# palantir/k8s-spark-scheduler

Hardware: AMD Instinct MI355X
Metric: gang-fit decisions/sec at 10k nodes x 1k pending apps (+ p99 Filter latency: fifo_filter) (higher is better)
Workload: dtype int64; 1 GPU; independent batch, tightly-pack, 10000 nodes x 1000 pending apps per GPU, 3-D (cpu milli, mem bytes, gpu) int64, SURVEY.md 8d/C2 distributions, seed 0x5EED0010; nodes=10000, apps_per_gpu=1000, algo=tightly-pack, mode=independent, batches_in_flight=11, regime=streamed_tickets (resident worker), backend=none, rccl_ranks=0

## Files before the change

### include/gangfit.h

```cpp
#ifndef GANGFIT_H
#define GANGFIT_H

#include <stddef.h>
#include <stdint.h>

#ifdef __cplusplus
extern "C" {
#endif

#define GF_VERSION 300

#define GF_OK 0
#define GF_ERR_NO_DEVICE (-1)
#define GF_ERR_HIP (-2)
#define GF_ERR_INVALID (-3)
#define GF_ERR_CAPACITY (-4)
#define GF_ERR_STATE (-5)
#define GF_ERR_UNSUPPORTED (-6)

#define GF_NO_NODE 0xFFFFFFFFu
#define GF_MAX_K (1 << 20)
#define GF_MAX_ABS_QUANTITY (INT64_C(1) << 62)

typedef enum gf_algo {
// ... 198 lines not shown

int gf_hbm_probe(gf_ctx *ctx, uint64_t bytes, uint32_t iters, double *read_gb_per_s, double *copy_gb_per_s);

int gf_launch_floor(gf_ctx *ctx, void *stream, uint32_t iters, float *us_per_launch);

typedef struct gf_worker_batch {
    uint32_t n_apps;
    uint32_t flags;
    const gf_app *d_apps;
    gf_result *d_results;
    uint32_t *d_exec_nodes;
    uint64_t exec_nodes_len;
} gf_worker_batch;
#define GF_WORKER_HOST_OUTPUTS 1u
#define GF_WORKER_LEAVE_AFTER 2u
int gf_worker_fit(gf_ctx *ctx, gf_algo algo, uint32_t n_apps, const gf_app *apps, gf_result *results, uint32_t *exec_nodes,
                  uint64_t exec_nodes_cap);
int gf_worker_submit_dev(gf_ctx *ctx, gf_algo algo, uint32_t n_batches, const gf_worker_batch *batches, uint64_t *first_ticket);
int gf_worker_wait(gf_ctx *ctx, uint64_t first_ticket, uint32_t n_tickets);
int gf_worker_stop(gf_ctx *ctx);
int gf_worker_stats(gf_ctx *ctx, uint64_t out[4]);
int gf_worker_geometry(gf_ctx *ctx, uint32_t out[2]);
int gf_worker_row_stats(gf_ctx *ctx, uint64_t out[3]);
int gf_call_phases(gf_ctx *ctx, double out_us[5]);
int gf_worker_kernel_time(gf_ctx *ctx, float *ms, uint64_t *tickets);

typedef struct gf_device_info {
    char name[128];
    char arch[64];
    int32_t compute_units;
    int32_t lds_bytes_per_cu;
    int32_t wavefront_size;
    int32_t clock_khz;
    int64_t hbm_bytes;
} gf_device_info;
int gf_device_info_get(gf_ctx *ctx, gf_device_info *out);

#ifdef __cplusplus
}
#endif
#endif
```

### k8s-spark-scheduler_amd/csrc/gangfit_api_worker.cpp

```cpp
#include "gangfit_ctx.h"

using namespace gfapi;

namespace gfapi {

constexpr uint32_t kRing = gangfit::kWorkerRing;

inline uint64_t host_load(const unsigned long long* p) { return __atomic_load_n(p, __ATOMIC_ACQUIRE); }
inline void host_store(unsigned long long* p, uint64_t v) { __atomic_store_n(p, (unsigned long long)v, __ATOMIC_RELEASE); }

int worker_alloc(gf_ctx* ctx) {
    gf_ctx::Worker& w = ctx->worker;
    if (w.allocated) return GF_OK;
    GF_HIP(ctx, hipSetDevice(ctx->device));
    void* hp = nullptr;
    GF_HIP(ctx, hipHostMalloc(&hp, sizeof(gangfit::WorkerHostCtl), hipHostMallocMapped | hipHostMallocCoherent));
    std::memset(hp, 0, sizeof(gangfit::WorkerHostCtl));
    void* hd = nullptr;
    if (hipHostGetDevicePointer(&hd, hp, 0) != hipSuccess) {
        (void)hipHostFree(hp);
        return fail(ctx, GF_ERR_HIP, "the worker's control block cannot be mapped to the device");
    }
    void* dp = nullptr;
    if (hipMalloc(&dp, sizeof(gangfit::WorkerDevCtl)) != hipSuccess ||
// ... 361 lines not shown
}

int gf_worker_geometry(gf_ctx* ctx, uint32_t out[2]) {
    if (!ctx || !out) return GF_ERR_INVALID;
    std::lock_guard<std::recursive_mutex> lock(ctx->mu);
    out[0] = ctx->worker.cur_sets;
    out[1] = ctx->worker.cur_blocks_per_set;
    return GF_OK;
}

int gf_worker_row_stats(gf_ctx* ctx, uint64_t out[3]) {
    if (!ctx || !out) return GF_ERR_INVALID;
    std::lock_guard<std::recursive_mutex> lock(ctx->mu);
    out[0] = out[1] = out[2] = 0;
    const gf_ctx::Worker& w = ctx->worker;
    if (!w.allocated) return GF_OK;
    GF_HIP(ctx, hipSetDevice(ctx->device));
    unsigned long long h[3] = {0, 0, 0};
    GF_HIP(ctx, hipMemcpy(h, w.d->rows, sizeof(h), hipMemcpyDeviceToHost));
    for (int i = 0; i < 3; ++i) out[i] = h[i];
    return GF_OK;
}

int gf_worker_kernel_time(gf_ctx* ctx, float* ms, uint64_t* tickets) {
    if (!ctx || !ms || !tickets) return GF_ERR_INVALID;
    std::lock_guard<std::recursive_mutex> lock(ctx->mu);
    const gf_ctx::Worker& w = ctx->worker;
    if (!w.allocated || w.launches == 0 || (w.running && w.launches == 1))
        return fail(ctx, GF_ERR_STATE, "no launch of the worker has finished yet (gf_worker_stop first)");
    if (!w.running) worker_elapsed(ctx->worker);
    *ms = w.last_ms;
    *tickets = w.last_tickets;
    return GF_OK;
}

}
```

### k8s-spark-scheduler_amd/csrc/gangfit_device.h

```cpp
#pragma once

#include <hip/hip_runtime.h>
#include <stdint.h>

#include <optional>

#include "gangfit.h"
#include "gangfit_worker_rounds.h"
#include "gangfit_worker_rows.h"

namespace gangfit {

struct NodeTable {
    int64_t* cpu;
    int64_t* mem;
    int64_t* gpu;
    const uint32_t* slot_node;
    const uint32_t* dslot;
    const uint32_t* node_slot;
    const int64_t* cmax;
    const uint64_t* xmask;
    const uint64_t* dmask;
    uint32_t n_chunks;
    uint32_t n_x;
// ... 96 lines not shown
constexpr uint32_t kWorkerInline = 16;
constexpr int kWorkerWaves = 16;
constexpr uint32_t kWorkerCountStride = 64;

struct WorkerTicket {
    unsigned long long word[8];
};
static_assert(sizeof(WorkerTicket) == 64, "one cache line per ticket");
__host__ __device__ inline unsigned long long worker_tag(unsigned long long ticket) { return ((ticket + 1ull) & 0x7FFFull) | 0x8000ull; }

struct WorkerHostCtl {
    unsigned long long posted;
    unsigned long long stop;
    unsigned long long pad0[6];
    unsigned long long consumed;
    unsigned long long state;
    unsigned long long pad1[6];
    unsigned long long done[kWorkerRing];
    WorkerTicket ring[kWorkerRing];
};

struct WorkerDevCtl {
    unsigned long long quit;
    unsigned long long rows[3];
    unsigned long long pad0[4];
    uint32_t count[kWorkerRing * kWorkerCountStride];
    WorkerTicket ring[kWorkerRing];
};

struct WorkerArgs {
    WorkerHostCtl* host;
    WorkerDevCtl* dev;
    unsigned long long generation;
    unsigned long long first_ticket;
    unsigned long long idle_ticks;
    unsigned long long leave_after;
    uint32_t* scratch;
    unsigned long long scratch_stride;
    uint32_t sets;
    uint32_t blocks_per_set;
    ScanStats* stats;
    uint32_t n_inline;
    uint32_t stride_mul;
    unsigned long long inline_words[kWorkerInline][6];
    ZoneTable zones;
    const int64_t* sched;
    uint32_t stride_shift;
    uint32_t pad_stride;
// ... 390 lines not shown
```

### k8s-spark-scheduler_amd/csrc/gangfit_worker.inc

```







__device__ __forceinline__ unsigned long long sys_load(const unsigned long long* p) {
    return __hip_atomic_load(p, __ATOMIC_RELAXED, __HIP_MEMORY_SCOPE_SYSTEM);
}
__device__ __forceinline__ void sys_store(unsigned long long* p, unsigned long long v) {
    __hip_atomic_store(p, v, __ATOMIC_RELAXED, __HIP_MEMORY_SCOPE_SYSTEM);
}

__device__ __forceinline__ App app_from_lanes(unsigned long long w) {
    App r;
    r.drv0 = (int64_t)read_lane((int64_t)w, 0);
    r.drv1 = (int64_t)read_lane((int64_t)w, 1);
    r.drv2 = (int64_t)read_lane((int64_t)w, 2);
    r.exe0 = (int64_t)read_lane((int64_t)w, 3);
    r.exe1 = (int64_t)read_lane((int64_t)w, 4);
    r.exe2 = (int64_t)read_lane((int64_t)w, 5);
    const uint64_t kf = (uint64_t)read_lane((int64_t)w, 6);
    r.k = (int32_t)(uint32_t)kf;
    r.flags = (uint32_t)(kf >> 32);
// ... 95 lines not shown
    r.node = read_lane(dnode, r.fl);
    r.found = true;
    return r;
}
static_assert(rows::kCapClamp == GF_MAX_K && rows::kRowLen == (uint32_t)kWave && rows::kRows <= (uint32_t)kWave, "lane = entry");

constexpr int kWorkerCounting = 100 + (int)GF_ALGO_TIGHTLY_PACK;
template <int WHICH>
__global__ __launch_bounds__(kWave* kWorkerWaves, 4) void fit_worker_kernel(NodeTable T, SparseTable G, WorkerArgs W) {
    constexpr int ALGO = WHICH == kWorkerCounting ? (int)GF_ALGO_TIGHTLY_PACK : WHICH;
    constexpr bool COUNT = WHICH != (int)GF_ALGO_TIGHTLY_PACK;
    constexpr bool kZoned = ALGO == GF_ALGO_SINGLE_AZ_TIGHTLY_PACK || ALGO == GF_ALGO_AZ_AWARE_TIGHTLY_PACK;
    constexpr int kInner = kZoned ? (int)GF_ALGO_TIGHTLY_PACK : ALGO;
    __shared__ uint32_t s_cnt[8];
    __shared__ uint32_t s_round[kWorkerWaves];
    __shared__ unsigned long long s_next[8];
    __shared__ unsigned long long s_g0[5][kWave];
    constexpr bool kNarrow = ALGO == GF_ALGO_TIGHTLY_PACK;
    __shared__ int32_t s_g0n[kNarrow ? 3 : 1][kWave];
    constexpr bool kRowsOn = WHICH == (int)GF_ALGO_TIGHTLY_PACK;
    constexpr uint32_t kRowsN = kRowsOn ? rows::kRows : 1u;
    struct RowsLds {
        uint32_t dir[kWave];
        int32_t key[3][kWave];
        uint32_t slot[kRowsN][kWave];
        uint32_t node[kRowsN][kWave];
        int32_t cap[kRowsN][kWave];
    };
    __shared__ RowsLds s_rows[1];
    __shared__ unsigned long long s_row_stat[3];
    __shared__ uint32_t s_left;
    const int lane = lane_id();
    const uint32_t wave = __builtin_amdgcn_readfirstlane(threadIdx.x >> 6);
    if (blockIdx.x == 0) {
        if (wave != 0) return;
        unsigned long long consumed = W.first_ticket;
        unsigned long long last = wall_clock64();
        if (lane == 0) sys_store(&W.host->state, 1ull);
        for (;;) {
            const unsigned long long posted = sys_load(&W.host->posted);
            const unsigned long long stop = sys_load(&W.host->stop);
            if (posted > consumed) {
                while (consumed < posted) {
                    unsigned long long w4[4];
#pragma unroll
                    for (int q = 0; q < 4; ++q) {
                        const unsigned long long t = consumed + (unsigned long long)(lane >> 3) + 8ull * (unsigned long long)q;
                        w4[q] = 0;
                        if (t < posted)
                            w4[q] = sys_load(reinterpret_cast<const unsigned long long*>(&W.host->ring[(uint32_t)(t % kWorkerRing)]) + (lane & 7));
                    }
#pragma unroll
                    for (int q = 0; q < 4; ++q) {
// ... 17 lines not shown
                }
                asm volatile("s_waitcnt vmcnt(0)" ::: "memory");
                if (lane == 0) sys_store(&W.host->state, 2ull);
                return;
            }
            __builtin_amdgcn_s_sleep(8);
        }
    }
    const uint32_t b = blockIdx.x - 1u;
    const uint32_t set = b / W.blocks_per_set, bs = b % W.blocks_per_set;
    const uint32_t app_stride = W.blocks_per_set * kWorkerWaves;
    const rounds::StrideDiv sdiv{W.stride_mul, W.stride_shift};
    unsigned long long t = W.first_ticket + (unsigned long long)((set + W.sets - (uint32_t)(W.first_ticket % W.sets)) % W.sets);
    GlobalView V{T.cpu, T.mem, T.gpu, T.cmax, T.cmax + T.n_chunks, T.cmax + 2 * (size_t)T.n_chunks, T.xmask, T.dmask,
                 T.n_chunks};
    Orders O{T.slot_node, T.dslot, T.n_x, T.n_d, T.d_identity != 0};
    const bool merged = T.d_identity != 0 && kInner != GF_ALGO_MINIMAL_FRAGMENTATION;
    constexpr uint32_t kCountSlots = 8;
    constexpr uint32_t kRoundGone = 0xFFFFFFFFu;
    if (threadIdx.x < kCountSlots) s_cnt[threadIdx.x] = 0;
    if (threadIdx.x < 8) s_next[threadIdx.x] = 0ull;
    if (threadIdx.x < (uint32_t)kWorkerWaves) s_round[threadIdx.x] = 0;
    if constexpr (kRowsOn) {
        if (threadIdx.x < kRowsN) s_rows[0].dir[threadIdx.x] = rows::kEmpty;
        if (threadIdx.x < 3) s_row_stat[threadIdx.x] = 0ull;
        if (threadIdx.x == 0) s_left = 0u;
    }
    const bool narrow_table = kNarrow && T.nquad != nullptr;
    bool rows_live = kRowsOn && merged &&
                           (W.leave_after == 0ull || W.leave_after - W.first_ticket >= (unsigned long long)rows::kRowSightings * W.sets);
    if (wave == 0) {
        const Group0 g = load_group0(V, O, lane);
        s_g0[0][lane] = (unsigned long long)g.m0;
        s_g0[1][lane] = (unsigned long long)g.m1;
        s_g0[2][lane] = (unsigned long long)g.m2;
        s_g0[3][lane] = g.dcand;
        s_g0[4][lane] = g.xcand;
        if constexpr (kNarrow) {
            if (narrow_table) {
                s_g0n[0][lane] = NarrowView::scale_max(g.m0, T.nunit[0]);
                s_g0n[1][lane] = NarrowView::scale_max(g.m1, T.nunit[1]);
                s_g0n[2][lane] = NarrowView::scale_max(g.m2, T.nunit[2]);
            }
        }
    }
    const NarrowView VN(InWorkerKernel{}, T.nquad, T.xmask, T.dmask, T.n_chunks);
    const int64_t unit_l = T.nunit[lane % 3 == 0 ? 0 : (lane % 3 == 1 ? 1 : 2)];
    const double rcp_l = kNarrow ? fast_rcp((double)unit_l) : 0.0;
    __syncthreads();
    constexpr bool kG0Regs = kNarrow;
    Group0T<int32_t> g0n_regs{};
    if constexpr (kG0Regs) {
        if (narrow_table) {
            g0n_regs.m0 = s_g0n[0][lane];
            g0n_regs.m1 = s_g0n[1][lane];
            g0n_regs.m2 = s_g0n[2][lane];
            g0n_regs.dcand = s_g0[3][lane];
            g0n_regs.xcand = s_g0[4][lane];
        }
    }
    typedef __attribute__((address_space(1))) const gf_app glb_app;
    typedef __attribute__((address_space(1))) gf_result glb_result;
    typedef __attribute__((address_space(1))) uint32_t glb_u32w;
    constexpr unsigned long long kPtrMask = 0x0000FFFFFFFFFFFFull;
    constexpr bool kRecords = ALGO != GF_ALGO_MINIMAL_FRAGMENTATION;
    auto load_words = [&](unsigned long long tt) {
        const unsigned long long* line = reinterpret_cast<const unsigned long long*>(&W.dev->ring[(uint32_t)(tt % kWorkerRing)]);
        unsigned long long w = 0;
        if (lane < 6) w = __hip_atomic_load(line + lane, __ATOMIC_RELAXED, __HIP_MEMORY_SCOPE_AGENT);
        return w;
    };
// ... 97 lines not shown
        uint32_t* scratch = priv + W.scratch_stride;
        const bool direct = ALGO == GF_ALGO_TIGHTLY_PACK && ((w5 >> 32) & 1ull) == 0;
        uint32_t mine = 0;
        for (uint32_t a = kRecords ? app_index(i_cur) : first_app; kRecords ? i_cur < total : a < n_apps;
             a = kRecords ? a : a + app_stride) {
            if constexpr (kRecords) {
                if (a >= n_apps) {
                    i_cur = grab(round);
                    a = app_index(i_cur);
                    if (i_cur < total && a < n_apps) wrec = load_record(apps, a);
                    continue;
                }
            }
            unsigned long long xvis = 0, dvis = 0;
            Decision dec;
            int32_t app_k = 0;
            uint64_t app_off = 0;
            bool decided = false;
            int build_row = -1;
            const uint32_t* placed = nullptr;
            if constexpr (kNarrow) {
                NarrowApp napp;
                auto sparse_serves = [&]() { return worker_kernargs_here()->G.n_x != 0u && O.d_identity; };
                if (narrow_table && scale_record(wrec, lane, unit_l, rcp_l, napp)) {
                if constexpr (kRowsOn) {
                    if (rows_live && napp.k > 0) {
                        RowsLds& R = s_rows[0];
                        int rl = lane;
                        GF_HERE(rl);
                        uint32_t st = rows::kEmpty;
                        bool same = false;
                        if ((uint32_t)rl < kRowsN) {
                            st = __hip_atomic_load(&R.dir[rl], __ATOMIC_ACQUIRE, __HIP_MEMORY_SCOPE_WORKGROUP);
                            const int32_t k0 = R.key[0][rl], k1 = R.key[1][rl], k2 = R.key[2][rl];
                            same = (bool)((int)rows::dir_has_key(st) & (int)(k0 == napp.exe0) & (int)(k1 == napp.exe1) & (int)(k2 == napp.exe2));
                        }
                        const uint64_t hit = __ballot(same);
                        bool served = false;
                        if (hit) {
                            const int e = __ffsll((unsigned long long)hit) - 1;
                            const uint32_t ste = read_lane(st, e);
                            if (rows::dir_ready(ste)) {
                                const RowDriver rd = wave_row_driver(VN, O, napp, g0n_regs, lane);
                                if (rd.found) {
                                    const int32_t c_ds = read_lane(cap3(rd.d0 - napp.drv0, rd.d1 - napp.drv1, rd.d2 - napp.drv2, napp), rd.fl);
                                    const int32_t cp = rows::entry_cap(R.slot[e][rl], R.cap[e][rl], rd.ds, c_ds);
                                    const uint32_t node = R.node[e][rl];
                                    const int32_t incl = wave_inclusive_scan(cp);
                                    if (rows::served((int64_t)read_lane(incl, kWave - 1), napp.k)) {
                                        const int64_t start = (int64_t)(incl - cp);
                                        emit_runs((direct ? exec_nodes : priv) + napp.exec_off, start, rows::run_of(start, cp, napp.k), node,
                                                  lane, direct);
                                        app_k = napp.k;
                                        app_off = napp.exec_off;
                                        dec.feasible = true;
                                        dec.ds = rd.ds;
                                        dec.pass1 = 0;
                                        dec.ds_node = rd.node;
                                        decided = served = true;
                                    }
                                }
                            } else if (rows::dir_counting(ste)) {
                                uint32_t old = 0;
                                if (lane == 0) old = __hip_atomic_fetch_add(&R.dir[e], 1u, __ATOMIC_RELAXED, __HIP_MEMORY_SCOPE_WORKGROUP);
                                if (rows::dir_sighting_builds((uint32_t)__builtin_amdgcn_readfirstlane(old))) build_row = e;
                            }
                        } else {
                            const uint64_t empty = __ballot((uint32_t)rl < kRowsN && st == rows::kEmpty);
                            const uint64_t claimed = __ballot(st == rows::kClaimed);
                            if (empty == 0ull && claimed == 0ull &&
                                __hip_atomic_load(&s_row_stat[0], __ATOMIC_RELAXED, __HIP_MEMORY_SCOPE_WORKGROUP) == 0ull)
                                rows_live = false;
                            if (empty != 0ull && claimed == 0ull && lane == 0) {
                                const int e = __ffsll((unsigned long long)empty) - 1;
                                uint32_t expect = rows::kEmpty;
                                if (__hip_atomic_compare_exchange_strong(&R.dir[e], &expect, rows::kClaimed, __ATOMIC_RELAXED, __ATOMIC_RELAXED,
                                                                         __HIP_MEMORY_SCOPE_WORKGROUP)) {
                                    R.key[0][e] = napp.exe0;
                                    R.key[1][e] = napp.exe1;
                                    R.key[2][e] = napp.exe2;
                                    __hip_atomic_store(&R.dir[e], rows::kFirstSighting, __ATOMIC_RELEASE, __HIP_MEMORY_SCOPE_WORKGROUP);
                                }
                            }
                        }
                        if (lane == 0)
                            __hip_atomic_fetch_add(&s_row_stat[served ? 1 : 2], 1ull, __ATOMIC_RELAXED, __HIP_MEMORY_SCOPE_WORKGROUP);
                    }
                }
                if (!decided && !(napp.exe2 > 0 && napp.k > 0 && sparse_serves())) {
                    Group0T<int32_t> g0n = g0n_regs;
                    if constexpr (!kG0Regs) {
                        g0n.m0 = s_g0n[0][lane];
                        g0n.m1 = s_g0n[1][lane];
                        g0n.m2 = s_g0n[2][lane];
                        g0n.dcand = s_g0[3][lane];
                        g0n.xcand = s_g0[4][lane];
                    }
                    app_k = napp.k;
                    app_off = napp.exec_off;
                    dec = wave_decide<ALGO, NarrowView, false>(VN, O, napp, (direct ? exec_nodes : priv) + app_off, scratch + app_off,
                                                               scratch + half + app_off, lane, xvis, dvis, &g0n, nullptr, direct);
                    if (dec.feasible && dec.ds_node == GF_NO_NODE) dec.ds_node = VN.node_of(dec.ds);
                    decided = true;
// ... 31 lines not shown
                }
            }
            if (dec.feasible && !direct) {
                if constexpr (kZoned) {
                    for (int32_t i = lane; i < app_k; i += kWave)
                        __hip_atomic_store(exec_nodes + app_off + i, T.slot_node[placed[i]], __ATOMIC_RELAXED, __HIP_MEMORY_SCOPE_SYSTEM);
                } else {
                    for (int32_t i = lane; i < app_k; i += kWave)
                        __hip_atomic_store(exec_nodes + app_off + i, priv[app_off + i], __ATOMIC_RELAXED,
                                           __HIP_MEMORY_SCOPE_SYSTEM);
                }
            }
            if (lane < 2) {
                if (dec.feasible && dec.ds_node == GF_NO_NODE) dec.ds_node = T.slot_node[dec.ds];
                const unsigned long long lo = (unsigned long long)(uint32_t)(dec.feasible ? 1 : 0) |
                                              ((unsigned long long)(dec.feasible ? dec.ds_node : GF_NO_NODE) << 32);
                const unsigned long long hi = (unsigned long long)(dec.feasible ? (uint32_t)app_k : 0u) | (1ull << 32);
                __hip_atomic_store(reinterpret_cast<unsigned long long*>(results + a) + lane, lane == 0 ? lo : hi, __ATOMIC_RELAXED,
                                   __HIP_MEMORY_SCOPE_SYSTEM);
            }
            if constexpr (kRowsOn) {
                if (__builtin_expect(build_row >= 0, 0)) {
                    NarrowApp b;
                    (void)scale_record(wrec, lane, unit_l, rcp_l, b);
                    b.k = rows::kCapClamp;
                    RowsLds& R = s_rows[0];
                    int rl = lane;
                    GF_HERE(rl);
                    R.slot[build_row][rl] = GF_NO_NODE;
                    R.node[build_row][rl] = GF_NO_NODE;
                    R.cap[build_row][rl] = 0;
                    const uint32_t xc = (O.n_x + kWave - 1) / kWave;
                    const uint64_t lt_mask = (1ull << lane) - 1ull;
                    uint32_t fill = 0;
                    for (uint32_t g = 0; g * kWave < xc && fill < rows::kRowLen; ++g) {
                        uint64_t cand;
                        uint64_t m = chunk_group_mask<false>(VN, g, xc, b.exe0, b.exe1, b.exe2, lane, cand);
                        while (m != 0ull && fill < rows::kRowLen) {
                            const int bit = __ffsll((unsigned long long)m) - 1;
                            const uint32_t c = g * kWave + (uint32_t)bit;
                            m &= m - 1;
                            const uint32_t j = c * kWave + lane;
                            const uint64_t in_m = (uint64_t)read_lane((int64_t)cand, bit) & low_lanes(chunk_len(O.n_x, c * kWave, kWave));
                            int32_t a0 = 0, a1 = 0, a2 = 0;
                            uint32_t node = 0;
                            if (lane_in(in_m)) VN.load(j, a0, a1, a2, node);
                            const uint64_t fm = ge3_mask(a0, a1, a2, b.exe0, b.exe1, b.exe2) & in_m;
                            const uint32_t pos = fill + (uint32_t)__popcll((unsigned long long)(fm & lt_mask));
                            if (lane_in(fm) && pos < rows::kRowLen) {
                                R.slot[build_row][pos] = j;
                                R.node[build_row][pos] = node;
                                R.cap[build_row][pos] = cap3(a0, a1, a2, b);
                            }
                            fill += (uint32_t)__popcll((unsigned long long)fm);
                        }
                    }
                    __builtin_amdgcn_fence(__ATOMIC_RELEASE, "workgroup");
                    if (lane == 0) {
                        __hip_atomic_fetch_add(&s_row_stat[0], 1ull, __ATOMIC_RELAXED, __HIP_MEMORY_SCOPE_WORKGROUP);
                        __hip_atomic_fetch_or(&R.dir[build_row], rows::kReadyBit, __ATOMIC_RELEASE, __HIP_MEMORY_SCOPE_WORKGROUP);
                    }
                }
            }
            ++mine;
            if constexpr (kRecords) {
                i_cur = grab(round);
                a = app_index(i_cur);
                if (i_cur < total && a < n_apps) wrec = load_record(apps, a);
            }
        }
        const unsigned long long t_next = t + W.sets;
        const bool have_next = words_valid(w_next, t_next);
        unsigned long long wrec_next = 0;
        uint32_t i_next = 0;
        const uint32_t bsr_n = rounds::next_block(bsr, W.blocks_per_set);
        const gf_app* apps_n = nullptr;
        uint64_t w5_n = 0;
        uint32_t rows_n = 0;
        if (kRecords && have_next) {
// ... 26 lines not shown
                            sys_store(&W.host->done[slot], t + 1ull);
                        }
                    }
                }
            }
        }
        ++round;
        if (lane == 0) __hip_atomic_store(&s_round[wave], round, __ATOMIC_RELAXED, __HIP_MEMORY_SCOPE_WORKGROUP);
        t = t_next;
        w_cur = w_next;
        have_cur = have_next;
        wrec = wrec_next;
        i_cur = i_next;
        grabbed_cur = kRecords && have_next;
        bsr = bsr_n;
        apps = apps_n;
        w5 = w5_n;
        rows = rows_n;
    }
    if (lane == 0) __hip_atomic_store(&s_round[wave], kRoundGone, __ATOMIC_RELAXED, __HIP_MEMORY_SCOPE_WORKGROUP);
    if constexpr (kRowsOn) {
        uint32_t left = 0;
        if (lane == 0) left = __hip_atomic_fetch_add(&s_left, 1u, __ATOMIC_ACQ_REL, __HIP_MEMORY_SCOPE_WORKGROUP);
        if ((uint32_t)__builtin_amdgcn_readfirstlane(left) == (uint32_t)kWorkerWaves - 1u && lane < 3) {
            const unsigned long long n = __hip_atomic_load(&s_row_stat[lane], __ATOMIC_RELAXED, __HIP_MEMORY_SCOPE_WORKGROUP);
            if (n != 0ull) __hip_atomic_fetch_add(&W.dev->rows[lane], n, __ATOMIC_RELAXED, __HIP_MEMORY_SCOPE_AGENT);
        }
    }
}
```

### k8s-spark-scheduler_amd/csrc/gangfit_worker_rows.h

```cpp
#pragma once
#include <cstdint>

#if defined(__HIPCC__)
#define GF_ROWS_FN __host__ __device__ inline
#else
#define GF_ROWS_FN inline
#endif

namespace gangfit {
namespace rows {

constexpr uint32_t kRowLen = 64;
constexpr uint32_t kRows = 40;
constexpr uint32_t kRowSightings = 4;
constexpr int32_t kCapClamp = 1 << 20;


constexpr uint32_t kEmpty = 0u, kClaimed = 1u, kFirstSighting = 2u, kReadyBit = 0x80000000u;
GF_ROWS_FN bool dir_ready(uint32_t w) { return (w & kReadyBit) != 0u; }
GF_ROWS_FN bool dir_has_key(uint32_t w) { return w >= kFirstSighting; }
GF_ROWS_FN bool dir_counting(uint32_t w) { return w >= kFirstSighting && w <= kRowSightings; }
GF_ROWS_FN bool dir_sighting_builds(uint32_t old) { return old == kRowSightings; }

GF_ROWS_FN int32_t entry_cap(uint32_t slot, int32_t cap, uint32_t ds, int32_t c_ds) { return slot == ds ? c_ds : cap; }
GF_ROWS_FN bool served(int64_t total, int32_t k) { return k >= 1 && total >= (int64_t)k; }
GF_ROWS_FN int32_t run_of(int64_t before, int32_t cap, int32_t k) {
    const int64_t room = (int64_t)k - before;
    return room <= 0 ? 0 : (room < (int64_t)cap ? (int32_t)room : cap);
}

GF_ROWS_FN bool decide(const uint32_t* slot, const uint32_t* node, const int32_t* cap, uint32_t n, uint32_t ds, int32_t c_ds,
                       int32_t k, uint32_t* out) {
    int64_t total = 0;
    for (uint32_t i = 0; i < n; ++i) total += entry_cap(slot[i], cap[i], ds, c_ds);
    if (!served(total, k)) return false;
    int64_t before = 0;
    for (uint32_t i = 0; i < n; ++i) {
        const int32_t c = entry_cap(slot[i], cap[i], ds, c_ds);
        const int32_t t = run_of(before, c, k);
        for (int32_t j = 0; j < t; ++j) out[before + j] = node[i];
        before += c;
    }
    return true;
}

}
}
```

### k8s-spark-scheduler_amd/gangfit/_native.py

```python
from __future__ import annotations

import ctypes as C
import os
import sys
from typing import Optional

import numpy as np

from . import build as _build

GF_OK = 0
GF_ERR_NO_DEVICE, GF_ERR_HIP, GF_ERR_INVALID, GF_ERR_CAPACITY, GF_ERR_STATE, GF_ERR_UNSUPPORTED = -1, -2, -3, -4, -5, -6
GF_NO_NODE = 0xFFFFFFFF
GF_MAX_K = 1 << 20
GF_ALGO_TIGHTLY_PACK = 0
GF_ALGO_DISTRIBUTE_EVENLY = 1
GF_ALGO_MINIMAL_FRAGMENTATION = 2
GF_ALGO_AZ_AWARE_TIGHTLY_PACK = 3
GF_ALGO_SINGLE_AZ_TIGHTLY_PACK = 4
GF_ALGO_SINGLE_AZ_MINIMAL_FRAGMENTATION = 5
GF_MODE_INDEPENDENT = 0
GF_MODE_FIFO_CHAIN = 1
GF_APP_SKIPPABLE = 1

# ... 1 lines not shown
    [("drv", "<i8", (3,)), ("exe", "<i8", (3,)), ("k", "<i4"), ("flags", "<u4"), ("exec_off", "<u8")], align=True
)
RESULT_DTYPE = np.dtype(
    [("has_capacity", "<i4"), ("driver_node", "<u4"), ("exec_len", "<u4"), ("evaluated", "<u4")], align=True
)
assert APP_DTYPE.itemsize == 64 and RESULT_DTYPE.itemsize == 16

GF_RESIDENT_USAGE = 0xFFFFFFFF
GF_ANY_ZONE = 0xFFFFFFFF
GF_WORKER_LEAVE_AFTER = 2
GF_EFF_AGAINST_SNAPSHOT = 0
GF_EFF_AGAINST_RESIDUAL = 1

EXPORTED_SYMBOLS = [
    "gf_version", "gf_init", "gf_destroy", "gf_last_error", "gf_snapshot_set", "gf_orders_set", "gf_fit_batch", "gf_fit_feasible",
    "gf_fit_batch_dev", "gf_spark_binpack", "gf_residual_get", "gf_timer_begin", "gf_timer_end", "gf_scan_stats", "gf_chain_profile",
    "gf_selftest", "gf_device_info_get", "gf_zones_set", "gf_avg_packing_efficiency", "gf_packing_efficiencies",
    "gf_hbm_probe", "gf_executor_fit", "gf_executor_fit_zoned", "gf_snapshot_build", "gf_snapshot_get", "gf_shard_set", "gf_shard_partials_dev", "gf_shard_drivers_dev", "gf_shard_emit_dev", "gf_shard_finish_dev",
    "gf_shard_layout", "gf_shard_mf_layout", "gf_shard_mf_counts_dev", "gf_shard_mf_drivers_dev", "gf_shard_mf_emit_dev",
    "gf_shard_mf_finish_dev",
    "gf_find_nodes", "gf_ctx_lock", "gf_ctx_unlock", "gf_launch_floor",
    "gf_graph_begin", "gf_graph_end", "gf_graph_launch", "gf_graph_destroy", "gf_cluster_set", "gf_snapshot_build_resident",
    "gf_usage_reset", "gf_usage_apply", "gf_overhead_update", "gf_set_option", "gf_chain_cache_stats", "gf_generation", "gf_shard_count", "gf_ctx_view",
    "gf_worker_fit", "gf_worker_submit_dev", "gf_worker_wait", "gf_worker_stop", "gf_worker_stats", "gf_worker_geometry", "gf_worker_row_stats", "gf_worker_kernel_time", "gf_call_phases",
    "gf_cluster_fit_feasible", "gf_cluster_fit_feasible_sets", "gf_snapshot_build_info", "gf_cluster_executor_fit",
    "gf_snapshot_build_resident_set", "gf_snapshot_set_info", "gf_filter_efficiency",
]


class DeviceInfo(C.Structure):
    _fields_ = [("name", C.c_char * 128), ("arch", C.c_char * 64), ("compute_units", C.c_int32),
                ("lds_bytes_per_cu", C.c_int32), ("wavefront_size", C.c_int32), ("clock_khz", C.c_int32),
                ("hbm_bytes", C.c_int64)]


class WorkerBatch(C.Structure):
    _fields_ = [("n_apps", C.c_uint32), ("flags", C.c_uint32), ("d_apps", C.c_void_p), ("d_results", C.c_void_p),
                ("d_exec_nodes", C.c_void_p), ("exec_nodes_len", C.c_uint64)]


GF_WORKER_HOST_OUTPUTS = 1


class GangfitError(RuntimeError):
    def __init__(self, code: int, message: str):
        super().__init__(f"libgangfit error {code}: {message}")
        self.code = code
# ... 114 lines not shown
    L.gf_scan_stats.argtypes = [p, i32, i32, p]
    L.gf_selftest.restype = i32
    L.gf_selftest.argtypes = [p, u64, u32, C.POINTER(u32)]
    L.gf_device_info_get.restype = i32
    L.gf_device_info_get.argtypes = [p, C.POINTER(DeviceInfo)]
    L.gf_set_option.restype = i32
    L.gf_set_option.argtypes = [p, C.c_char_p, C.c_int64]
    L.gf_ctx_view.restype = i32
    L.gf_ctx_view.argtypes = [p, C.POINTER(p)]
    L.gf_worker_fit.restype = i32
    L.gf_worker_fit.argtypes = [p, i32, u32, p, p, p, u64]
    L.gf_worker_submit_dev.restype = i32
    L.gf_worker_submit_dev.argtypes = [p, i32, u32, p, p]
    L.gf_worker_wait.restype = i32
    L.gf_worker_wait.argtypes = [p, u64, u32]
    L.gf_worker_stop.restype = i32
    L.gf_worker_stop.argtypes = [p]
    L.gf_worker_stats.restype = i32
    L.gf_worker_stats.argtypes = [p, p]
    L.gf_worker_geometry.restype = i32
    L.gf_worker_geometry.argtypes = [p, p]
    L.gf_worker_row_stats.restype = i32
    L.gf_worker_row_stats.argtypes = [p, p]
    L.gf_fit_feasible.restype = i32
    L.gf_fit_feasible.argtypes = [p, i32, u32, p, p]
    L.gf_cluster_fit_feasible.restype = i32
    L.gf_cluster_fit_feasible.argtypes = [p, i32, p, p, p, p, u32, p, p]
    L.gf_cluster_fit_feasible_sets.restype = i32
    L.gf_cluster_fit_feasible_sets.argtypes = [p, i32, p, p, p, u32, p, p, u32, p, p]
    L.gf_cluster_executor_fit.restype = i32
    L.gf_cluster_executor_fit.argtypes = [p, i32, u32, p, u32, p, p, p, p, p, p, p]
    L.gf_chain_profile.restype = i32
    L.gf_chain_profile.argtypes = [p, p]
    L.gf_call_phases.restype = i32
    L.gf_call_phases.argtypes = [p, C.POINTER(C.c_double)]
    L.gf_worker_kernel_time.restype = i32
    L.gf_worker_kernel_time.argtypes = [p, C.POINTER(C.c_float), C.POINTER(C.c_uint64)]
    L.gf_shard_count.restype = i32
    L.gf_shard_count.argtypes = [p]
    L.gf_generation.restype = i32
    L.gf_generation.argtypes = [p, p]
    L.gf_chain_cache_stats.restype = i32
    L.gf_chain_cache_stats.argtypes = [p, i32, p]
    L.gf_snapshot_build_info.restype = i32
    L.gf_snapshot_build_info.argtypes = [p, p]
    L.gf_snapshot_build_resident_set.restype = i32
# ... 10 lines not shown
```

### k8s-spark-scheduler_amd/gangfit/context.py

```python
from __future__ import annotations

import ctypes as C
from dataclasses import dataclass
from typing import Optional, Tuple

import numpy as np

from . import _native as N


def make_apps(drv, exe, k, flags=None) -> np.ndarray:
    drv = np.asarray(drv, dtype=np.int64).reshape(-1, 3)
    exe = np.asarray(exe, dtype=np.int64).reshape(-1, 3)
    k = np.asarray(k, dtype=np.int32).reshape(-1)
    apps = np.zeros(len(k), dtype=N.APP_DTYPE)
    apps["drv"], apps["exe"], apps["k"] = drv, exe, k
    if flags is not None:
        apps["flags"] = np.asarray(flags, dtype=np.uint32)
    return apps


def with_offsets(apps: np.ndarray) -> Tuple[np.ndarray, int]:
    apps = apps.copy()
    k = np.clip(apps["k"].astype(np.int64), 0, None).astype(np.uint64)
# ... 450 lines not shown
        return int(first.value)

    def worker_wait(self, first_ticket: int, n_tickets: int = 1):
        self._check(self._lib.gf_worker_wait(self._h, first_ticket, n_tickets))

    def worker_stop(self):
        self._check(self._lib.gf_worker_stop(self._h))

    def worker_stats(self):
        out = (C.c_uint64 * 4)()
        self._check(self._lib.gf_worker_stats(self._h, out))
        return {"posted": int(out[0]), "complete": int(out[1]), "launches": int(out[2]), "resident": bool(out[3])}

    def worker_geometry(self):
        out = (C.c_uint32 * 2)()
        self._check(self._lib.gf_worker_geometry(self._h, out))
        return int(out[0]), int(out[1])

    def worker_row_stats(self):
        out = (C.c_uint64 * 3)()
        self._check(self._lib.gf_worker_row_stats(self._h, out))
        return {"built": int(out[0]), "served": int(out[1]), "fell_back": int(out[2])}

    def call_phases(self):
        out = (C.c_double * 5)()
        self._check(self._lib.gf_call_phases(self._h, out))
        return {"stage": out[0], "launch": out[1], "wait": out[2], "copy_out": out[3], "total": out[4]}

    def worker_kernel_time(self):
        ms, n = C.c_float(), C.c_uint64()
        self._check(self._lib.gf_worker_kernel_time(self._h, C.byref(ms), C.byref(n)))
        return float(ms.value), int(n.value)

    def graph_begin(self, stream: int = 0):
        self._check(self._lib.gf_graph_begin(self._h, C.c_void_p(stream) if stream else None))

    def graph_end(self, stream: int = 0) -> int:
        g = C.c_void_p()
        self._check(self._lib.gf_graph_end(self._h, C.c_void_p(stream) if stream else None, C.byref(g)))
        return g.value

    def graph_launch(self, graph: int, stream: int = 0):
        self._check(self._lib.gf_graph_launch(self._h, C.c_void_p(graph), C.c_void_p(stream) if stream else None))

    def graph_destroy(self, graph: int):
        self._lib.gf_graph_destroy(self._h, C.c_void_p(graph))
# ... 58 lines not shown
```

Before: 1.392 billion decisions/s.

## Memoize driver-slot placement per driver request in worker LDS row directory

Extends the per-workgroup LDS row cache so directory lanes beyond the executor rows hold driver-request memo entries. Each entry stores the driver residual, driver slot and node, and executor rows now also keep magic-division payloads. A repeated (driver, executor) shape can then be decided from LDS with a multiply-shift capacity computation, skipping app scaling and the driver scan. The per-lane reciprocal moves into shared memory, and new counters are exposed through a stats API. The cost is extra LDS footprint, more ballots and compares on every probe, and a fallback path whenever the memo cannot serve a request.

```diff
diff --git a/include/gangfit.h b/include/gangfit.h
--- a/include/gangfit.h
+++ b/include/gangfit.h
@@ -244,6 +244,7 @@
 int gf_worker_stats(gf_ctx *ctx, uint64_t out[4]);
 int gf_worker_geometry(gf_ctx *ctx, uint32_t out[2]);
 int gf_worker_row_stats(gf_ctx *ctx, uint64_t out[3]);
+int gf_worker_memo_stats(gf_ctx *ctx, uint64_t out[2]);
 int gf_call_phases(gf_ctx *ctx, double out_us[5]);
 int gf_worker_kernel_time(gf_ctx *ctx, float *ms, uint64_t *tickets);
 
diff --git a/k8s-spark-scheduler_amd/csrc/gangfit_api_worker.cpp b/k8s-spark-scheduler_amd/csrc/gangfit_api_worker.cpp
--- a/k8s-spark-scheduler_amd/csrc/gangfit_api_worker.cpp
+++ b/k8s-spark-scheduler_amd/csrc/gangfit_api_worker.cpp
@@ -407,6 +407,19 @@
     return GF_OK;
 }
 
+int gf_worker_memo_stats(gf_ctx* ctx, uint64_t out[2]) {
+    if (!ctx || !out) return GF_ERR_INVALID;
+    std::lock_guard<std::recursive_mutex> lock(ctx->mu);
+    out[0] = out[1] = 0;
+    const gf_ctx::Worker& w = ctx->worker;
+    if (!w.allocated) return GF_OK;
+    GF_HIP(ctx, hipSetDevice(ctx->device));
+    unsigned long long h[2] = {0, 0};
+    GF_HIP(ctx, hipMemcpy(h, w.d->rows + 3, sizeof(h), hipMemcpyDeviceToHost));
+    for (int i = 0; i < 2; ++i) out[i] = h[i];
+    return GF_OK;
+}
+
 int gf_worker_kernel_time(gf_ctx* ctx, float* ms, uint64_t* tickets) {
     if (!ctx || !ms || !tickets) return GF_ERR_INVALID;
     std::lock_guard<std::recursive_mutex> lock(ctx->mu);
diff --git a/k8s-spark-scheduler_amd/csrc/gangfit_device.h b/k8s-spark-scheduler_amd/csrc/gangfit_device.h
--- a/k8s-spark-scheduler_amd/csrc/gangfit_device.h
+++ b/k8s-spark-scheduler_amd/csrc/gangfit_device.h
@@ -142,8 +142,8 @@
 
 struct WorkerDevCtl {
     unsigned long long quit;
-    unsigned long long rows[3];
-    unsigned long long pad0[4];
+    unsigned long long rows[5];
+    unsigned long long pad0[2];
     uint32_t count[kWorkerRing * kWorkerCountStride];
     WorkerTicket ring[kWorkerRing];
 };
diff --git a/k8s-spark-scheduler_amd/csrc/gangfit_worker.inc b/k8s-spark-scheduler_amd/csrc/gangfit_worker.inc
--- a/k8s-spark-scheduler_amd/csrc/gangfit_worker.inc
+++ b/k8s-spark-scheduler_amd/csrc/gangfit_worker.inc
@@ -1,3 +1,4 @@
+
 
 
 
@@ -141,13 +142,15 @@
     constexpr uint32_t kRowsN = kRowsOn ? rows::kRows : 1u;
     struct RowsLds {
         uint32_t dir[kWave];
-        int32_t key[3][kWave];
+        unsigned long long key[kRowsOn ? 3 : 1][kWave];
+        uint32_t pay[kRowsOn ? kWave : 1][8];
         uint32_t slot[kRowsN][kWave];
         uint32_t node[kRowsN][kWave];
         int32_t cap[kRowsN][kWave];
     };
     __shared__ RowsLds s_rows[1];
-    __shared__ unsigned long long s_row_stat[3];
+    __shared__ unsigned long long s_row_stat[5];
+    __shared__ double s_rcp[kNarrow ? kWave : 1];
     __shared__ uint32_t s_left;
     const int lane = lane_id();
     const uint32_t wave = __builtin_amdgcn_readfirstlane(threadIdx.x >> 6);
@@ -211,13 +214,13 @@
     if (threadIdx.x < 8) s_next[threadIdx.x] = 0ull;
     if (threadIdx.x < (uint32_t)kWorkerWaves) s_round[threadIdx.x] = 0;
     if constexpr (kRowsOn) {
-        if (threadIdx.x < kRowsN) s_rows[0].dir[threadIdx.x] = rows::kEmpty;
-        if (threadIdx.x < 3) s_row_stat[threadIdx.x] = 0ull;
+        if (threadIdx.x < (uint32_t)kWave) s_rows[0].dir[threadIdx.x] = rows::kEmpty;
+        if (threadIdx.x < 5) s_row_stat[threadIdx.x] = 0ull;
         if (threadIdx.x == 0) s_left = 0u;
     }
     const bool narrow_table = kNarrow && T.nquad != nullptr;
-    bool rows_live = kRowsOn && merged &&
-                           (W.leave_after == 0ull || W.leave_after - W.first_ticket >= (unsigned long long)rows::kRowSightings * W.sets);
+    int look = (kRowsOn && merged &&
+                (W.leave_after == 0ull || W.leave_after - W.first_ticket >= (unsigned long long)rows::kRowSightings * W.sets)) ? 2 : 0;
     if (wave == 0) {
         const Group0 g = load_group0(V, O, lane);
         s_g0[0][lane] = (unsigned long long)g.m0;
@@ -235,7 +238,14 @@
     }
     const NarrowView VN(InWorkerKernel{}, T.nquad, T.xmask, T.dmask, T.n_chunks);
     const int64_t unit_l = T.nunit[lane % 3 == 0 ? 0 : (lane % 3 == 1 ? 1 : 2)];
-    const double rcp_l = kNarrow ? fast_rcp((double)unit_l) : 0.0;
+    if constexpr (kNarrow) {
+        if (wave == 0) s_rcp[lane] = fast_rcp((double)unit_l);
+    }
+    auto scale_here = [&](unsigned long long w, NarrowApp& r) {
+        int sl = lane;
+        GF_HERE(sl);
+        return scale_record(w, lane, unit_l, s_rcp[sl], r);
+    };
     __syncthreads();
     constexpr bool kG0Regs = kNarrow;
     Group0T<int32_t> g0n_regs{};
@@ -379,28 +389,96 @@
             if constexpr (kNarrow) {
                 NarrowApp napp;
                 auto sparse_serves = [&]() { return worker_kernargs_here()->G.n_x != 0u && O.d_identity; };
-                if (narrow_table && scale_record(wrec, lane, unit_l, rcp_l, napp)) {
+                int pe = -1, pd = -1;
+                uint32_t ste = rows::kEmpty, stdr = rows::kEmpty;
+                uint64_t m_empty = 0ull, m_claimed = 0ull;
+                bool probed = false, memo_fell = false;
                 if constexpr (kRowsOn) {
-                    if (rows_live && napp.k > 0) {
+                    if (look != 0 && narrow_table) {
                         RowsLds& R = s_rows[0];
                         int rl = lane;
                         GF_HERE(rl);
-                        uint32_t st = rows::kEmpty;
-                        bool same = false;
-                        if ((uint32_t)rl < kRowsN) {
-                            st = __hip_atomic_load(&R.dir[rl], __ATOMIC_ACQUIRE, __HIP_MEMORY_SCOPE_WORKGROUP);
-                            const int32_t k0 = R.key[0][rl], k1 = R.key[1][rl], k2 = R.key[2][rl];
-                            same = (bool)((int)rows::dir_has_key(st) & (int)(k0 == napp.exe0) & (int)(k1 == napp.exe1) & (int)(k2 == napp.exe2));
+                        const uint32_t st = __hip_atomic_load(&R.dir[rl], __ATOMIC_ACQUIRE, __HIP_MEMORY_SCOPE_WORKGROUP);
+                        const unsigned long long k0 = R.key[0][rl], k1 = R.key[1][rl], k2 = R.key[2][rl];
+                        constexpr int kEQ = 32;
+                        const uint64_t same_x = __builtin_amdgcn_uicmpl((unsigned long)k0, (unsigned long)read_lane((int64_t)wrec, 3), kEQ) &
+                                                __builtin_amdgcn_uicmpl((unsigned long)k1, (unsigned long)read_lane((int64_t)wrec, 4), kEQ) &
+                                                __builtin_amdgcn_uicmpl((unsigned long)k2, (unsigned long)read_lane((int64_t)wrec, 5), kEQ);
+                        uint64_t same_d = 0ull;
+                        if (look == 2)
+                            same_d = __builtin_amdgcn_uicmpl((unsigned long)k0, (unsigned long)read_lane((int64_t)wrec, 0), kEQ) &
+                                     __builtin_amdgcn_uicmpl((unsigned long)k1, (unsigned long)read_lane((int64_t)wrec, 1), kEQ) &
+                                     __builtin_amdgcn_uicmpl((unsigned long)k2, (unsigned long)read_lane((int64_t)wrec, 2), kEQ);
+                        const uint64_t hit = rows::key_hits(__ballot(rows::dir_has_key(st)), same_x, same_d);
+                        m_empty = __ballot(rows::memo_claimable(st));
+                        m_claimed = __ballot(st == rows::kClaimed);
+                        probed = true;
+                        if ((hit & low_lanes(rows::kRows)) != 0ull) {
+                            pe = __ffsll((unsigned long long)(hit & low_lanes(rows::kRows))) - 1;
+                            ste = read_lane(st, pe);
                         }
-                        const uint64_t hit = __ballot(same);
+                        if ((hit >> rows::kRows) != 0ull) {
+                            pd = __ffsll((unsigned long long)(hit >> rows::kRows)) - 1 + (int)rows::kRows;
+                            stdr = read_lane(st, pd);
+                        }
+                        const int32_t rk = (int32_t)(uint32_t)(uint64_t)read_lane((int64_t)wrec, 6);
+                        if (pe >= 0 && pd >= 0 && rows::memo_qualifies(ste, stdr, rk)) {
+                            uint32_t dw = 0, mg = 0, su = 0;
+                            if (rl < 5) dw = R.pay[pd][rl];
+                            if (rl < 3) {
+                                mg = R.pay[pe][rl];
+                                su = R.pay[pe][3 + rl];
+                            }
+                            const uint32_t q = rows::memo_quot((int32_t)dw, mg, su);
+                            const bool neg = __ballot(rl < 3 && (int32_t)dw < 0) != 0ull;
+                            const int32_t c_ds = rows::memo_cap_of(read_lane(q, 0), read_lane(q, 1), read_lane(q, 2), neg, rk);
+                            const uint32_t ds = read_lane(dw, 3), dnode = read_lane(dw, 4);
+                            const int32_t cp = rows::entry_cap(R.slot[pe][rl], R.cap[pe][rl], ds, c_ds);
+                            const uint32_t node = R.node[pe][rl];
+                            const int32_t incl = wave_inclusive_scan(cp);
+                            const bool srv = rows::served((int64_t)read_lane(incl, kWave - 1), rk);
+                            if (srv) {
+                                const uint64_t off = (uint64_t)read_lane((int64_t)wrec, 7);
+                                const int64_t start = (int64_t)(incl - cp);
+                                emit_runs((direct ? exec_nodes : priv) + off, start, rows::run_of(start, cp, rk), node, lane, direct);
+                                app_k = rk;
+                                app_off = off;
+                                dec.feasible = true;
+                                dec.ds = ds;
+                                dec.pass1 = 0;
+                                dec.ds_node = dnode;
+                                decided = true;
+                            } else {
+                                memo_fell = true;
+                            }
+                            if (lane == 0)
+                                __hip_atomic_fetch_add(&s_row_stat[srv ? 4 : 2], 1ull, __ATOMIC_RELAXED, __HIP_MEMORY_SCOPE_WORKGROUP);
+                        }
+                    }
+                }
+                if (!decided && narrow_table && scale_here(wrec, napp)) {
+                if constexpr (kRowsOn) {
+                    if (probed && napp.k > 0 && !memo_fell) {
+                        RowsLds& R = s_rows[0];
+                        int rl = lane;
+                        GF_HERE(rl);
                         bool served = false;
-                        if (hit) {
-                            const int e = __ffsll((unsigned long long)hit) - 1;
-                            const uint32_t ste = read_lane(st, e);
+                        if (pe >= 0) {
+                            const int e = pe;
                             if (rows::dir_ready(ste)) {
                                 const RowDriver rd = wave_row_driver(VN, O, napp, g0n_regs, lane);
                                 if (rd.found) {
                                     const int32_t c_ds = read_lane(cap3(rd.d0 - napp.drv0, rd.d1 - napp.drv1, rd.d2 - napp.drv2, napp), rd.fl);
+                                    if (look == 2 && pd < 0 && ((m_empty | m_claimed) >> rows::kRows) == 0ull &&
+                                        __hip_atomic_load(&s_row_stat[4], __ATOMIC_RELAXED, __HIP_MEMORY_SCOPE_WORKGROUP) == 0ull)
+                                        look = 1;
+                                    const bool fill = look == 2 && pd < 0 && (m_empty >> rows::kRows) != 0ull && (m_claimed >> rows::kRows) == 0ull;
+                                    int32_t q0 = 0, q1 = 0, q2 = 0;
+                                    if (fill) {
+                                        q0 = read_lane(rd.d0 - napp.drv0, rd.fl);
+                                        q1 = read_lane(rd.d1 - napp.drv1, rd.fl);
+                                        q2 = read_lane(rd.d2 - napp.drv2, rd.fl);
+                                    }
                                     const int32_t cp = rows::entry_cap(R.slot[e][rl], R.cap[e][rl], rd.ds, c_ds);
                                     const uint32_t node = R.node[e][rl];
                                     const int32_t incl = wave_inclusive_scan(cp);
@@ -416,6 +494,28 @@
                                         dec.ds_node = rd.node;
                                         decided = served = true;
                                     }
+                                    if (fill) {
+                                        const int de = __ffsll((unsigned long long)(m_empty >> rows::kRows)) - 1 + (int)rows::kRows;
+                                        const unsigned long long x0 = (unsigned long long)read_lane((int64_t)wrec, 0);
+                                        const unsigned long long x1 = (unsigned long long)read_lane((int64_t)wrec, 1);
+                                        const unsigned long long x2 = (unsigned long long)read_lane((int64_t)wrec, 2);
+                                        if (lane == 0) {
+                                            uint32_t expect = rows::kEmpty;
+                                            if (__hip_atomic_compare_exchange_strong(&R.dir[de], &expect, rows::kClaimed, __ATOMIC_RELAXED,
+                                                                                     __ATOMIC_RELAXED, __HIP_MEMORY_SCOPE_WORKGROUP)) {
+                                                R.key[0][de] = x0;
+                                                R.key[1][de] = x1;
+                                                R.key[2][de] = x2;
+                                                R.pay[de][0] = (uint32_t)q0;
+                                                R.pay[de][1] = (uint32_t)q1;
+                                                R.pay[de][2] = (uint32_t)q2;
+                                                R.pay[de][3] = rd.ds;
+                                                R.pay[de][4] = rd.node;
+                                                __hip_atomic_store(&R.dir[de], rows::kMemoReady, __ATOMIC_RELEASE, __HIP_MEMORY_SCOPE_WORKGROUP);
+                                                __hip_atomic_fetch_add(&s_row_stat[3], 1ull, __ATOMIC_RELAXED, __HIP_MEMORY_SCOPE_WORKGROUP);
+                                            }
+                                        }
+                                    }
                                 }
                             } else if (rows::dir_counting(ste)) {
                                 uint32_t old = 0;
@@ -423,19 +523,22 @@
                                 if (rows::dir_sighting_builds((uint32_t)__builtin_amdgcn_readfirstlane(old))) build_row = e;
                             }
                         } else {
-                            const uint64_t empty = __ballot((uint32_t)rl < kRowsN && st == rows::kEmpty);
-                            const uint64_t claimed = __ballot(st == rows::kClaimed);
+                            const uint64_t empty = m_empty & low_lanes(rows::kRows);
+                            const uint64_t claimed = m_claimed & low_lanes(rows::kRows);
                             if (empty == 0ull && claimed == 0ull &&
                                 __hip_atomic_load(&s_row_stat[0], __ATOMIC_RELAXED, __HIP_MEMORY_SCOPE_WORKGROUP) == 0ull)
-                                rows_live = false;
-                            if (empty != 0ull && claimed == 0ull && lane == 0) {
+                                look = 0;
+                            if (empty != 0ull && claimed == 0ull) {
+                                const unsigned long long x0 = (unsigned long long)read_lane((int64_t)wrec, 3);
+                                const unsigned long long x1 = (unsigned long long)read_lane((int64_t)wrec, 4);
+                                const unsigned long long x2 = (unsigned long long)read_lane((int64_t)wrec, 5);
                                 const int e = __ffsll((unsigned long long)empty) - 1;
                                 uint32_t expect = rows::kEmpty;
-                                if (__hip_atomic_compare_exchange_strong(&R.dir[e], &expect, rows::kClaimed, __ATOMIC_RELAXED, __ATOMIC_RELAXED,
-                                                                         __HIP_MEMORY_SCOPE_WORKGROUP)) {
-                                    R.key[0][e] = napp.exe0;
-                                    R.key[1][e] = napp.exe1;
-                                    R.key[2][e] = napp.exe2;
+                                if (lane == 0 && __hip_atomic_compare_exchange_strong(&R.dir[e], &expect, rows::kClaimed, __ATOMIC_RELAXED,
+                                                                                      __ATOMIC_RELAXED, __HIP_MEMORY_SCOPE_WORKGROUP)) {
+                                    R.key[0][e] = x0;
+                                    R.key[1][e] = x1;
+                                    R.key[2][e] = x2;
                                     __hip_atomic_store(&R.dir[e], rows::kFirstSighting, __ATOMIC_RELEASE, __HIP_MEMORY_SCOPE_WORKGROUP);
                                 }
                             }
@@ -513,7 +616,7 @@
             if constexpr (kRowsOn) {
                 if (__builtin_expect(build_row >= 0, 0)) {
                     NarrowApp b;
-                    (void)scale_record(wrec, lane, unit_l, rcp_l, b);
+                    (void)scale_here(load_record(apps, a), b);
                     b.k = rows::kCapClamp;
                     RowsLds& R = s_rows[0];
                     int rl = lane;
@@ -546,6 +649,14 @@
                             fill += (uint32_t)__popcll((unsigned long long)fm);
                         }
                     }
+                    if (lane == 0) {
+                        R.pay[build_row][0] = b.mag0;
+                        R.pay[build_row][1] = b.mag1;
+                        R.pay[build_row][2] = b.mag2;
+                        R.pay[build_row][3] = rows::pack_su(b.sh0, b.exe0 == 0);
+                        R.pay[build_row][4] = rows::pack_su(b.sh1, b.exe1 == 0);
+                        R.pay[build_row][5] = rows::pack_su(b.sh2, b.exe2 == 0);
+                    }
                     __builtin_amdgcn_fence(__ATOMIC_RELEASE, "workgroup");
                     if (lane == 0) {
                         __hip_atomic_fetch_add(&s_row_stat[0], 1ull, __ATOMIC_RELAXED, __HIP_MEMORY_SCOPE_WORKGROUP);
@@ -618,9 +729,12 @@
     if constexpr (kRowsOn) {
         uint32_t left = 0;
         if (lane == 0) left = __hip_atomic_fetch_add(&s_left, 1u, __ATOMIC_ACQ_REL, __HIP_MEMORY_SCOPE_WORKGROUP);
-        if ((uint32_t)__builtin_amdgcn_readfirstlane(left) == (uint32_t)kWorkerWaves - 1u && lane < 3) {
+        if ((uint32_t)__builtin_amdgcn_readfirstlane(left) == (uint32_t)kWorkerWaves - 1u && lane < 5) {
             const unsigned long long n = __hip_atomic_load(&s_row_stat[lane], __ATOMIC_RELAXED, __HIP_MEMORY_SCOPE_WORKGROUP);
-            if (n != 0ull) __hip_atomic_fetch_add(&W.dev->rows[lane], n, __ATOMIC_RELAXED, __HIP_MEMORY_SCOPE_AGENT);
-        }
-    }
-}
+            if (n != 0ull) {
+                __hip_atomic_fetch_add(&W.dev->rows[lane], n, __ATOMIC_RELAXED, __HIP_MEMORY_SCOPE_AGENT);
+                if (lane == 4) __hip_atomic_fetch_add(&W.dev->rows[1], n, __ATOMIC_RELAXED, __HIP_MEMORY_SCOPE_AGENT);
+            }
+        }
+    }
+}
diff --git a/k8s-spark-scheduler_amd/csrc/gangfit_worker_rows.h b/k8s-spark-scheduler_amd/csrc/gangfit_worker_rows.h
--- a/k8s-spark-scheduler_amd/csrc/gangfit_worker_rows.h
+++ b/k8s-spark-scheduler_amd/csrc/gangfit_worker_rows.h
@@ -22,6 +22,31 @@
 GF_ROWS_FN bool dir_counting(uint32_t w) { return w >= kFirstSighting && w <= kRowSightings; }
 GF_ROWS_FN bool dir_sighting_builds(uint32_t old) { return old == kRowSightings; }
 
+constexpr uint32_t kDrivers = 24;
+static_assert(kRows + kDrivers == kRowLen, "one directory lane per entry");
+constexpr uint32_t kMemoReady = kReadyBit;
+GF_ROWS_FN bool memo_claimable(uint32_t w) { return w == kEmpty; }
+GF_ROWS_FN bool memo_ready(uint32_t w) { return dir_ready(w); }
+constexpr uint64_t kExeLanes = (1ull << kRows) - 1ull;
+GF_ROWS_FN uint64_t key_hits(uint64_t has_key, uint64_t same_exe, uint64_t same_drv) {
+    return has_key & ((same_exe & kExeLanes) | (same_drv & ~kExeLanes));
+}
+GF_ROWS_FN bool memo_qualifies(uint32_t exe_word, uint32_t drv_word, int32_t k) {
+    return dir_ready(exe_word) && memo_ready(drv_word) && k >= 1 && k <= kCapClamp;
+}
+GF_ROWS_FN uint32_t pack_su(uint32_t sh, bool zero_request) { return sh | ((uint32_t)zero_request << 8); }
+GF_ROWS_FN uint32_t mulhi32(uint32_t a, uint32_t b) { return (uint32_t)(((uint64_t)a * (uint64_t)b) >> 32); }
+GF_ROWS_FN uint32_t memo_quot(int32_t a, uint32_t mag, uint32_t su) { return (mulhi32(mag, (uint32_t)a << 1) >> (su & 31u)) | (0u - (su >> 8)); }
+GF_ROWS_FN int32_t memo_cap_of(uint32_t q0, uint32_t q1, uint32_t q2, bool any_negative, int32_t k) {
+    uint32_t q = q0 < q1 ? q0 : q1;
+    q = q < q2 ? q : q2;
+    q = q < (uint32_t)k ? q : (uint32_t)k;
+    return any_negative ? 0 : (int32_t)q;
+}
+GF_ROWS_FN int32_t memo_cap(const int32_t a[3], const uint32_t mag[3], const uint32_t su[3], int32_t k) {
+    return memo_cap_of(memo_quot(a[0], mag[0], su[0]), memo_quot(a[1], mag[1], su[1]), memo_quot(a[2], mag[2], su[2]), (a[0] | a[1] | a[2]) < 0, k);
+}
+
 GF_ROWS_FN int32_t entry_cap(uint32_t slot, int32_t cap, uint32_t ds, int32_t c_ds) { return slot == ds ? c_ds : cap; }
 GF_ROWS_FN bool served(int64_t total, int32_t k) { return k >= 1 && total >= (int64_t)k; }
 GF_ROWS_FN int32_t run_of(int64_t before, int32_t cap, int32_t k) {
@@ -44,5 +69,10 @@
     return true;
 }
 
+GF_ROWS_FN bool memo_decide(const uint32_t* slot, const uint32_t* node, const int32_t* cap, uint32_t n, uint32_t ds, const int32_t residual[3],
+                            const uint32_t mag[3], const uint32_t su[3], int32_t k, uint32_t* out) {
+    return decide(slot, node, cap, n, ds, memo_cap(residual, mag, su, k), k, out);
+}
+
 }
 }
diff --git a/k8s-spark-scheduler_amd/gangfit/_native.py b/k8s-spark-scheduler_amd/gangfit/_native.py
--- a/k8s-spark-scheduler_amd/gangfit/_native.py
+++ b/k8s-spark-scheduler_amd/gangfit/_native.py
@@ -47,7 +47,7 @@
     "gf_find_nodes", "gf_ctx_lock", "gf_ctx_unlock", "gf_launch_floor",
     "gf_graph_begin", "gf_graph_end", "gf_graph_launch", "gf_graph_destroy", "gf_cluster_set", "gf_snapshot_build_resident",
     "gf_usage_reset", "gf_usage_apply", "gf_overhead_update", "gf_set_option", "gf_chain_cache_stats", "gf_generation", "gf_shard_count", "gf_ctx_view",
-    "gf_worker_fit", "gf_worker_submit_dev", "gf_worker_wait", "gf_worker_stop", "gf_worker_stats", "gf_worker_geometry", "gf_worker_row_stats", "gf_worker_kernel_time", "gf_call_phases",
+    "gf_worker_fit", "gf_worker_submit_dev", "gf_worker_wait", "gf_worker_stop", "gf_worker_stats", "gf_worker_geometry", "gf_worker_row_stats", "gf_worker_memo_stats", "gf_worker_kernel_time", "gf_call_phases",
     "gf_cluster_fit_feasible", "gf_cluster_fit_feasible_sets", "gf_snapshot_build_info", "gf_cluster_executor_fit",
     "gf_snapshot_build_resident_set", "gf_snapshot_set_info", "gf_filter_efficiency",
 ]
@@ -208,6 +208,8 @@
     L.gf_worker_geometry.argtypes = [p, p]
     L.gf_worker_row_stats.restype = i32
     L.gf_worker_row_stats.argtypes = [p, p]
+    L.gf_worker_memo_stats.restype = i32
+    L.gf_worker_memo_stats.argtypes = [p, p]
     L.gf_fit_feasible.restype = i32
     L.gf_fit_feasible.argtypes = [p, i32, u32, p, p]
     L.gf_cluster_fit_feasible.restype = i32
diff --git a/k8s-spark-scheduler_amd/gangfit/context.py b/k8s-spark-scheduler_amd/gangfit/context.py
--- a/k8s-spark-scheduler_amd/gangfit/context.py
+++ b/k8s-spark-scheduler_amd/gangfit/context.py
@@ -496,6 +496,11 @@
         self._check(self._lib.gf_worker_row_stats(self._h, out))
         return {"built": int(out[0]), "served": int(out[1]), "fell_back": int(out[2])}
 
+    def worker_memo_stats(self):
+        out = (C.c_uint64 * 2)()
+        self._check(self._lib.gf_worker_memo_stats(self._h, out))
+        return {"filled": int(out[0]), "served": int(out[1])}
+
     def call_phases(self):
         out = (C.c_double * 5)()
         self._check(self._lib.gf_call_phases(self._h, out))
```

New measurement: 1.676 billion decisions/s, median of 6. 20.5% higher.
